# naver/deep-image-retrieval

Measured on AMD Instinct MI355X. Metric: images/sec descriptor extraction (resnet101-GeM, 1024x1024), higher is better.
Workload: dtype fp16p

## Files before the change

### deep-image-retrieval_amd/csrc/c_api.hip

```cpp
#include <initializer_list>
#include <new>

#include "engine.h"
#include "pointwise.h"

namespace dir {
const char* last_error();
}
using namespace dir;

static constexpr int kSimSplitMinRows = 32768;

#define DIR_TRY try {
#define DIR_CATCH                                                   \
    }                                                               \
    catch (const std::bad_alloc&) {                                 \
        return fail(DIR_ERR_NOMEM, "out of host memory");           \
    }                                                               \
    catch (const std::exception& ex) {                              \
        return fail(DIR_ERR_INVALID, std::string("exception: ") + ex.what()); \
    }                                                               \
    catch (...) {                                                   \
        return fail(DIR_ERR_INVALID, "unknown exception");          \
    }
// ... 418 lines not shown
    if (a.ksplit > 1 && conv_splitk_bytes(a, a.ksplit) > scratch_bytes)
        return fail(DIR_ERR_WORKSPACE, "conv: split-K scratch too small");
    if (ksplit_used) *ksplit_used = a.ksplit > 1 ? a.ksplit : 1;
    return conv_launch(a, dtype, variant, (hipStream_t)stream);
    DIR_CATCH
}

static int launch_c3c1(const char* who, const ConvArgs& a, int dtype, void* stream, std::initializer_list<const void*> tensors) {
    for (const void* q : tensors)
        if ((uintptr_t)q & 15) return fail(DIR_ERR_INVALID, std::string(who) + ": tensors must be 16-byte aligned");
    hipError_t e = conv_c3c1_launch(a, dtype, (hipStream_t)stream);
    if (e != hipSuccess) return fail(DIR_ERR_HIP, std::string(who) + " launch: " + hipGetErrorString(e));
    return DIR_OK;
}

int dir_conv_c3c1(const void* t2, const void* w3, const float* bias3, const void* res, void* y, const void* w1,
                  const float* bias1, void* t1, int B, int H, int W, int P, int P2, int relu3, int relu1, int dtype,
                  void* stream) {
    DIR_TRY
    ConvArgs a;
    DIR_CHECK(fill_conv_args(a, t2, w3, bias3, res, y, B, H, W, P, 4 * P, 1, 1, 1, 0, H, W, relu3));
    if (!w1 || !bias1 || !t1 || !res) return fail(DIR_ERR_INVALID, "conv_c3c1: null pointer");
    if (dtype != DIR_BF16 && dtype != DIR_FP16) return fail(DIR_ERR_INVALID, "conv_c3c1: bad dtype");
    conv_args_next_conv1(a, (const uint16_t*)w1, nullptr, bias1, (uint16_t*)t1, P2, relu1 ? 1 : 0);
    if (!conv_c3c1_admissible(a))
        return fail(DIR_ERR_INVALID, "conv_c3c1: planes must be 64, 128 (P2 = P, or 128 after 64) or 256 (P2 = 256, B*H*W % 64 == 0)");
    return launch_c3c1("conv_c3c1", a, dtype, stream, {t2, w3, res, y, w1, t1, bias3, bias1});
    DIR_CATCH
}

int dir_conv_c3c1_ds(const void* t2, const void* x, const void* wcat, const float* bias, void* y, const void* w1,
                     const float* bias1, void* t1, int B, int H, int W, int relu3, int relu1, int dtype,
                     void* stream) {
    DIR_TRY
    ConvArgs a;
    DIR_CHECK(fill_conv_args(a, t2, wcat, bias, nullptr, y, B, H, W, 64, 256, 1, 1, 1, 0, H, W, relu3));
    if (!x || !w1 || !bias1 || !t1) return fail(DIR_ERR_INVALID, "conv_c3c1_ds: null pointer");
    if (dtype != DIR_BF16 && dtype != DIR_FP16) return fail(DIR_ERR_INVALID, "conv_c3c1_ds: bad dtype");
    a.x2 = (const uint16_t*)x;
    a.Cin2 = 64;
    conv_args_next_conv1(a, (const uint16_t*)w1, nullptr, bias1, (uint16_t*)t1, 64, relu1 ? 1 : 0);
    if (!conv_c3c1_admissible(a)) return fail(DIR_ERR_INVALID, "conv_c3c1_ds: shape not admissible");
    return launch_c3c1("conv_c3c1_ds", a, dtype, stream, {t2, x, wcat, y, w1, t1, bias, bias1});
    DIR_CATCH
}

int dir_conv_c3c1_wpair(const void* t2, const void* w3, const void* w3_lo, const float* bias3, const void* res, void* y,
                        const void* w1, const void* w1_lo, const float* bias1, void* t1, int B, int H, int W, int P2,
                        int relu3, int relu1, void* stream) {
    DIR_TRY
    ConvArgs a;
    DIR_CHECK(fill_conv_args(a, t2, w3, bias3, res, y, B, H, W, 64, 256, 1, 1, 1, 0, H, W, relu3));
    if (!w3_lo || !w1 || !bias1 || !t1 || !res) return fail(DIR_ERR_INVALID, "conv_c3c1_wpair: null pointer");
    a.w_lo = (const uint16_t*)w3_lo;
    conv_args_next_conv1(a, (const uint16_t*)w1, (const uint16_t*)w1_lo, bias1, (uint16_t*)t1, P2, relu1 ? 1 : 0);
    if (!conv_c3c1_admissible(a))
        return fail(DIR_ERR_INVALID, "conv_c3c1_wpair: planes 64; P2 = 64 (w1_lo required) or 128 (w1_lo optional)");
    return launch_c3c1("conv_c3c1_wpair", a, DIR_FP16, stream, {t2, w3, w3_lo, res, y, w1, w1_lo, t1, bias3, bias1});
    DIR_CATCH
}

int dir_conv_c3c1_ds_wpair(const void* t2, const void* x, const void* x_lo, const void* wcat, const void* wcat_lo,
                           const float* bias, void* y, const void* w1, const void* w1_lo, const float* bias1, void* t1,
                           int B, int H, int W, int relu3, int relu1, void* stream) {
    DIR_TRY
    ConvArgs a;
    DIR_CHECK(fill_conv_args(a, t2, wcat, bias, nullptr, y, B, H, W, 64, 256, 1, 1, 1, 0, H, W, relu3));
    if (!x || !x_lo || !wcat_lo || !w1 || !w1_lo || !bias1 || !t1) return fail(DIR_ERR_INVALID, "conv_c3c1_ds_wpair: null pointer");
    a.x2 = (const uint16_t*)x;
    a.x2_lo = (const uint16_t*)x_lo;
    a.Cin2 = 64;
    a.w_lo = (const uint16_t*)wcat_lo;
    conv_args_next_conv1(a, (const uint16_t*)w1, (const uint16_t*)w1_lo, bias1, (uint16_t*)t1, 64, relu1 ? 1 : 0);
// ... 473 lines not shown
```

### deep-image-retrieval_amd/csrc/conv_c3c1.hip

```cpp
#include "dir_common.h"
#include "conv_device.h"
#include "conv_igemm.h"

namespace dir {

template <class DT, int P, bool DS, int P2, bool WP3 = false, bool WP1 = false>
__global__ void __launch_bounds__(512) conv_c3c1_kernel(const ConvArgs a) {
    static_assert(P == 64 || P == 128, "planes");
    static_assert(P2 == P || (P == 64 && P2 == 128), "conv1' width");
    static_assert(!DS || (P == 64 && P2 == 64), "the downsample form is layer1's: 64 + 64 input channels");
    static_assert((!WP3 && !WP1) || P == 64, "paired weights: layer1's seams");
    constexpr int KW = P + (DS ? 64 : 0);
    constexpr int KA = KW + (DS && WP3 ? 64 : 0);
    constexpr int C4 = 4 * P;
    constexpr int BM = 64, NT = 512;
    constexpr int CW = C4 / 8;
    constexpr int TA = CW / 32;
    constexpr int KSA = KA / 16;
    constexpr int KSW = KW / 16;
    constexpr int XBUF = BM * KA * 2;
    constexpr int NX = XBUF / 16 / NT;
    constexpr int EROW = 32 * 4 + 16;
    constexpr int EPI_OFF = 2 * XBUF;
    constexpr int OUT_OFF = EPI_OFF + 8 * 32 * EROW;
// ... 103 lines not shown

    u32x4_t xr[NX];
    load_x(tile, xr);
    int cur = 0;
    u32x4_t rres0[TA * 2], rres1[TA * 2];
    if (!DS) load_res(tile, 0, rres0);
    store_x(xr, smem);
    __syncthreads();
    for (;;) {
        const bool more = tile + per < mt;
        const int next = more ? tile + per : tile;
        load_x(next, xr);
        const int m0 = tile * BM;
        if (!DS) load_res(tile, 1, rres1);
        const char* xb = smem + cur * XBUF;

#pragma unroll
        for (int j = 0; j < 2; ++j) {
            f32x16_t acc[TA];
#pragma unroll
            for (int i = 0; i < TA; ++i)
#pragma unroll
                for (int e = 0; e < 16; ++e) acc[i][e] = 0.f;
#pragma unroll
            for (int ks = 0; ks < KSA; ++ks) {
                const frag_t xf = *(const frag_t*)(xb + (ks >> 2) * (BM * 128) + j * (32 * 128) + lbase +
                                                   (((2 * (ks & 3) + lhi) ^ lswz) << 4));
                const int kw = ks < KSW ? ks : ks - 4;
#pragma unroll
                for (int i = 0; i < TA; ++i) {
// ... 25 lines not shown
#pragma unroll
                for (int pass = 0; pass < 2; ++pass) {
                    const int mrow = pass * 16 + erow;
                    const f32x4_t f0 = *(const f32x4_t*)(ebase + mrow * EROW + ecol * 4);
                    const f32x4_t f1 = *(const f32x4_t*)(ebase + mrow * EROW + ecol * 4 + 16);
                    float v[8] = {f0[0] + b0[0], f0[1] + b0[1], f0[2] + b0[2], f0[3] + b0[3],
                                  f1[0] + b1[0], f1[1] + b1[1], f1[2] + b1[2], f1[3] + b1[3]};
                    if (!DS) {
                        const u32x4_t rv = j == 0 ? rres0[i * 2 + pass] : rres1[i * 2 + pass];
                        add_res8<DT>(v, rv);
                    }
                    if (a.relu) relu8(v);
                    u32x4_t ov;
#pragma unroll
                    for (int e = 0; e < 4; ++e) ov[e] = DT::pack(v[2 * e], v[2 * e + 1]);
                    __builtin_amdgcn_raw_buffer_store_b128(ov, rsrc_y, row_off(m0 + j * 32 + mrow), i * 64, 0);
                    ovf.see(ov);
                    const int n = n_wave + i * 32 + ecol, p = j * 32 + mrow;
                    *(u32x4_t*)(otile + (n >> 6) * (BM * 128) + p * 128 + ((((n & 63) >> 3) ^ ((p >> 1) & 7)) << 4)) = ov;
                }
                wave_lds_sync();
            }
            if (!DS && j == 0) load_res(next, 0, rres0);
        }
        __syncthreads();

        {
            constexpr int NJ = WIDE ? 2 : 1;
            f32x16_t acc1[NJ];
#pragma unroll
            for (int jj = 0; jj < NJ; ++jj)
#pragma unroll
                for (int e = 0; e < 16; ++e) acc1[jj][e] = 0.f;
// ... 58 lines not shown
                    ovf.see(ov);
                }
            }
        }
        if (!more) break;
        store_x(xr, smem + (cur ^ 1) * XBUF);
        tile = next;
        cur ^= 1;
        __syncthreads();
    }
    ovf.flush(a.ovf);
}

bool conv_c3c1_admissible(const ConvArgs& a) {
    const bool ds = a.x2 != nullptr;
#ifdef DIR_EXPERIMENTS
    if (a.Cin == 256) return conv_seam3_admissible(a);
#endif
    return a.R == 1 && a.S == 1 && a.stride == 1 && a.pad == 0 && a.H == a.OH && a.W == a.OW &&
           (a.Cin == 64 || a.Cin == 128) && a.Cout == 4 * a.Cin && (ds ? (a.res == nullptr && a.Cin == 64 && a.Cin2 == 64)
                                                                       : a.res != nullptr) &&
           a.w2 != nullptr && a.bias2 != nullptr && a.y2 != nullptr &&
           (a.Cout2 == a.Cin || (!ds && a.Cin == 64 && a.Cout2 == 128)) && (long)a.M * a.Cout < (1L << 30) &&
           ((!a.w_lo && !a.w2_lo && !a.x2_lo) ||
            (a.Cin == 64 && a.w_lo && (a.w2_lo || a.Cout2 == 128) && (ds ? a.x2_lo != nullptr : a.x2_lo == nullptr)));
}

template <class DT, int P, bool DS, int P2 = P, bool WP3 = false, bool WP1 = false>
static hipError_t launch_c3c1(const ConvArgs& a, hipStream_t stream) {
    constexpr int XBUF = 64 * (P + (DS ? 64 : 0) + (DS && WP3 ? 64 : 0)) * 2;
    constexpr int LDS = 2 * XBUF + 8 * 32 * (32 * 4 + 16) + 64 * 4 * P * 2 + (4 * P + P2) * 4;
    static_assert(LDS <= 160 * 1024, "LDS budget");
    auto kern = conv_c3c1_kernel<DT, P, DS, P2, WP3, WP1>;
    static std::atomic<uint64_t> attr_done{0};
    if (hipError_t e = ensure_dynamic_lds((const void*)kern, LDS, attr_done); e != hipSuccess) return e;
    ConvArgs b = a;
    b.x_bytes = (uint32_t)((size_t)a.M * a.Cin * 2);
    const int mt = (a.M + 63) / 64;
    const int ncu = cu_count();
    hipLaunchKernelGGL(kern, dim3(mt < ncu ? mt : ncu), dim3(512), LDS, stream, b);
    return hipGetLastError();
}

hipError_t conv_c3c1_launch(const ConvArgs& a, int dtype, hipStream_t stream) {
#ifdef DIR_EXPERIMENTS
    if (a.Cin == 256) return conv_seam3_launch(a, dtype, stream);
#endif
    if (a.x2 && !env().no_c3c1lc && conv_c3c1ds_lc_admissible(a)) return conv_c3c1ds_lc_launch(a, dtype, stream);
    if (a.w_lo) {
        if (dtype != DIR_FP16) return hipErrorInvalidValue;
        if (a.x2) return a.w2_lo ? launch_c3c1<FP16, 64, true, 64, true, true>(a, stream) : hipErrorInvalidValue;
        if (a.Cout2 == 128)
// ... 15 lines not shown
```

### deep-image-retrieval_amd/csrc/conv_igemm.h

```cpp
#pragma once
#include "dir_common.h"

namespace dir {

struct ConvArgs {
    const uint16_t* x;
    const uint16_t* w;
    const float* bias;
    const uint16_t* res;
    uint16_t* y;
    int B, H, W, Cin, OH, OW, Cout;
    int R, S, stride, pad, relu;
    int M;
    int Ktot;
    int T;
    int ksplit;
    float* partial;
    const uint16_t* w2;
    const float* bias2;
    uint16_t* y2;
    int Cout2, relu2;
    const uint16_t* x2;
    int Cin2;
    int H2, W2, stride2;
// ... 2 lines not shown
    const uint16_t* x_lo;
    const uint16_t* x2_lo;
    const uint16_t* w_lo;
    const uint16_t* w_pw;
    const uint16_t* w_s2;
    const uint16_t* w2_lo;
    const uint16_t* res_lo;
    uint16_t* y_lo;
    int tiles_m, tiles_n;
    uint32_t x_bytes, w_bytes;
    int rev_m;
    int no_xcd_map;
    int flat;
    uint32_t div_ohw_mul, div_ohw_shr;
    uint32_t div_ow_mul, div_ow_shr;
};

inline void fastdiv_init(uint32_t d, uint32_t& mul, uint32_t& shr) {
    if (d <= 1) {
        mul = 0;
        shr = 0;
        return;
    }
    uint32_t l = 0;
    while ((1ull << l) < d) ++l;
    mul = (uint32_t)(((1ull << (31 + l)) + d - 1) / d);
    shr = l - 1;
}

inline void conv_fill_extents(ConvArgs& b) {
// ... 125 lines not shown
```

### deep-image-retrieval_amd/csrc/dir_common.h

```cpp
#pragma once
#include <hip/hip_runtime.h>
#include <stdint.h>
#include <string.h>
#include <atomic>
#include <string>

#include "../../include/dir_engine.h"

namespace dir {

typedef __attribute__((ext_vector_type(8))) __bf16 bf16x8_t;
typedef __attribute__((ext_vector_type(8))) _Float16 f16x8_t;
typedef __attribute__((ext_vector_type(16))) float f32x16_t;
typedef __attribute__((ext_vector_type(4))) float f32x4_t;
typedef __attribute__((ext_vector_type(4))) uint32_t u32x4_t;
typedef __attribute__((ext_vector_type(2))) uint32_t u32x2_t;
typedef __attribute__((ext_vector_type(4))) int i32x4_t;
typedef __attribute__((ext_vector_type(16))) int i32x16_t;
typedef __attribute__((ext_vector_type(2))) float f32x2_t;
typedef __attribute__((ext_vector_type(2))) __bf16 bf16x2_t;
typedef __attribute__((ext_vector_type(2))) _Float16 f16x2_t;

#define DIR_GLOBAL __attribute__((address_space(1)))
#define DIR_LDS __attribute__((address_space(3)))
// ... 23 lines not shown
    bool patchw_pack = false, no_patchw_pack = false;
    bool small_k2 = false;
    bool no_patchs2 = false;
    bool x3_k2048 = false;
    bool lc1x1 = false;
    bool no_c3c1lc = false;
    bool no_smallmap = false;
    bool no_wregd = false;
    bool no_patchw_lc = false;
    bool no_xcdmap = false;
    bool no_pair_patch = false, pair_acts = false;
    int pair_stages = 1;
    bool sim_v1 = false, sim_exact = false;
    bool experiments = false;
    bool no_inplace = false;
    bool no_stem_u8 = false;
    bool stem_pair_old = false;
    bool stem_u8_prep = false;
    bool stem_u8_wg8 = false;
    int stem_u8_seg = 0;
};
const Env& env();
void reload_env();

__host__ __device__ inline uint16_t f32_to_bf16_bits(float f) {
    uint32_t u;
    memcpy(&u, &f, 4);
    if ((u & 0x7fffffffu) > 0x7f800000u) return (uint16_t)((u >> 16) | 0x40);
    u += 0x7fffu + ((u >> 16) & 1u);
    return (uint16_t)(u >> 16);
// ... 149 lines not shown
```

### deep-image-retrieval_amd/csrc/engine.h

```cpp
#pragma once
#include <map>
#include <string>
#include <vector>

#include "conv_f32.h"
#include "conv_igemm.h"
#include "pointwise.h"

namespace dir {

struct HostTensor {
    std::vector<int64_t> shape;
    std::vector<float> data;
};

struct ConvLayer {
    std::string name;
    std::string wkey;
    std::string bnprefix;
    int Cin = 0, Cout = 0, R = 1, S = 1, stride = 1, pad = 0;
    bool relu = false;
    bool stem = false;
    struct Dev {
        uint16_t* w = nullptr;
// ... 88 lines not shown
                int* fh, int* fw, int* fc, void* ws, size_t ws_bytes, hipStream_t stream);
    int forward_f32(const void* img, int B, int H, int W, int fmt, float* desc_out, void* feat_out, int* fh, int* fw,
                    int* fc, char* base, const dir::Plan& p, hipStream_t stream);
    int run_conv_f32(dir::ConvLayer& L, const float* x, const float* res, float* y, int B, int H, int W, int OH, int OW,
                     hipStream_t stream);
    int run_conv(dir::ConvLayer& L, const uint16_t* x, const uint16_t* res, uint16_t* y, int B,
                 int H, int W, int OH, int OW, hipStream_t stream, bool rev_m = false);
    int run_conv_pair(dir::ConvLayer& L, const uint16_t* x, const uint16_t* x_lo, const uint16_t* res,
                      const uint16_t* res_lo, uint16_t* y, uint16_t* y_lo, int B, int H, int W, int OH, int OW,
                      hipStream_t stream, const uint16_t* x2 = nullptr, const uint16_t* x2_lo = nullptr);
    int forward_pair_head(const void* img, int B, int H, int W, int fmt, char* base, const dir::Plan& p,
                          hipStream_t stream, uint16_t** cur, int* h, int* w, size_t* next_block);
    int forward_pair_stem(const void* img, int B, int H, int W, int fmt, char* base, const dir::Plan& p, hipStream_t stream);
    bool pick_seam(const dir::ConvLayer& c3, const dir::ConvLayer& c1, const uint16_t* t2, const uint16_t* res, uint16_t* y,
                   uint16_t* t1, int B, int H, int W, const uint16_t* block_in, const uint16_t* block_in_lo,
                   dir::ConvArgs* a) const;
    int run_seam(const dir::ConvLayer& c3, const dir::ConvLayer& c1, const dir::ConvArgs& a, hipStream_t stream);
    int pick_conv_dual(const dir::ConvLayer& c3, const dir::ConvLayer& ds, const uint16_t* t2, const uint16_t* xin,
                       uint16_t* y, int B, int Hin, int Win, int OH, int OW, dir::ConvArgs* a) const;
    int run_conv_dual(const dir::ConvLayer& c3, const dir::ConvLayer& ds, const dir::ConvArgs& a, int variant,
                      hipStream_t stream);
    int tune_conv(dir::ConvLayer& L, dir::ConvArgs& a, hipStream_t stream, int* variant);
    int finish_descriptor(float* pooled, float* fcout, int B, float* desc_out, hipStream_t stream);
    dir::Env sw;
    float* splitk_scratch = nullptr;
    bool recording() const { return profiling && !prof_paused; }
    int prof_slot(dir::ProfSlot** slot);
    template <class Label, class Launch>
    int profiled(Label&& label, double flops, double bytes, hipStream_t stream, Launch&& launch) {
        if (!recording()) return launch();
        dir::ProfSlot* s = nullptr;
// ... 18 lines not shown
```

### deep-image-retrieval_amd/csrc/engine.hip

```cpp
#include "engine.h"

#include <math.h>
#include <algorithm>

namespace dir {

static thread_local std::string g_err;
void set_error(const std::string& msg) { g_err = msg; }
int fail(int code, const std::string& msg) {
    g_err = msg;
    return code;
}
const char* last_error() { return g_err.c_str(); }


static Env read_env() {
    Env e;
    auto on = [](const char* k) { return getenv(k) != nullptr; };
    const char* mode = getenv("DIRTORCH_AMD_C3C1");
    e.c3c1_off = mode && mode[0] == '0';
    e.c3c1_force = mode && mode[0] == 'f';
    e.no_ds_seam = on("DIRTORCH_AMD_NO_DS_SEAM");
    e.no_dual = on("DIRTORCH_AMD_NO_DUAL");
    e.rev_conv1 = on("DIRTORCH_AMD_REV_CONV1");
// ... 11 lines not shown
    e.small_k2 = on("DIRTORCH_AMD_SMALL_K2");
    e.patchw_pack = on("DIRTORCH_AMD_PATCHW_PACK");
    e.no_patchw_pack = on("DIRTORCH_AMD_NO_PATCHW_PACK");
    e.no_patchw = on("DIRTORCH_AMD_NO_PATCHW");
    e.no_x3 = on("DIRTORCH_AMD_NO_X3");
    e.no_patchs = on("DIRTORCH_AMD_NO_PATCHS");
    e.no_patchw_lc = on("DIRTORCH_AMD_NO_PATCHW_LC");
    e.no_xcdmap = on("DIRTORCH_AMD_NO_XCDMAP");
    e.no_pair_patch = on("DIRTORCH_AMD_NO_PAIR_PATCH");
    e.pair_acts = on("DIRTORCH_AMD_PAIR_ACTS");
    if (const char* s = getenv("DIRTORCH_AMD_PAIR_STAGES")) e.pair_stages = atoi(s);
    e.sim_v1 = on("DIRTORCH_AMD_SIM_V1");
    e.sim_exact = on("DIRTORCH_AMD_SIM_EXACT");
    e.experiments = on("DIRTORCH_AMD_EXPERIMENTS");
    e.no_inplace = on("DIRTORCH_AMD_NO_INPLACE");
    e.no_stem_u8 = on("DIRTORCH_AMD_NO_STEM_U8");
    e.stem_u8_wg8 = on("DIRTORCH_AMD_STEM_U8_WG8");
    e.stem_u8_prep = on("DIRTORCH_AMD_STEM_U8_PREP");
    e.stem_pair_old = on("DIRTORCH_AMD_STEM_PAIR_OLD");
    if (const char* s = getenv("DIRTORCH_AMD_STEM_U8_SEG")) e.stem_u8_seg = atoi(s);
    return e;
}
static Env g_env[2];
static std::atomic<int> g_env_cur{-1};
static std::atomic_flag g_env_lock = ATOMIC_FLAG_INIT;
static void publish_env() {
    while (g_env_lock.test_and_set(std::memory_order_acquire)) {
    }
    const int cur = g_env_cur.load(std::memory_order_relaxed);
    const int nxt = cur < 0 ? 0 : 1 - cur;
// ... 584 lines not shown
        h = oh;
        w = ow;
    }
    *cur_out = pp[cur];
    *h_out = h;
    *w_out = w;
    *next_block = nb;
    return DIR_OK;
}

static constexpr long kSeamMinTiles = 2048;
static constexpr long kSeam3MinTiles = 768;

bool dir_engine::pick_seam(const ConvLayer& c3, const ConvLayer& c1, const uint16_t* t2, const uint16_t* res, uint16_t* y,
                           uint16_t* t1, int B, int H, int W, const uint16_t* block_in, const uint16_t* block_in_lo,
                           ConvArgs* ap) const {
    ConvArgs& a = *ap;
    if (sw.c3c1_off) return false;
    conv_args_init(a, layer_geom(c3, B, H, W, H, W), t2, c3.dev.w, c3.dev.bias, res, y);
    a.w_lo = c3.dev.w_lo;
    if (block_in) {
        if (!c3.dev.w_ds || c3.Cin != 64) return false;
        a.w = c3.dev.w_ds;
        a.w_lo = c3.dev.w_ds_lo;
        a.bias = c3.dev.bias_ds;
        a.res = nullptr;
        a.x2 = block_in;
        a.x2_lo = block_in_lo;
        a.Cin2 = 64;
        if ((c3.dev.w_lo != nullptr) != (a.w_lo != nullptr)) return false;
    }
    conv_args_next_conv1(a, c1.dev.w, c1.dev.w_lo, c1.dev.bias, t1, c1.Cout, c1.relu ? 1 : 0);
    a.ovf = dev.ovf;
    if (c1.R != 1 || c1.S != 1 || c1.stride != 1 || c1.pad != 0 || c1.Cin != c3.Cout || !conv_c3c1_admissible(a))
        return false;
    if (!sw.c3c1_force && (a.M + 63) / 64 < (a.Cin == 256 ? kSeam3MinTiles : kSeamMinTiles)) return false;
    if (a.Cin == 256 && !sw.experiments) return false;
    return true;
}

int dir_engine::run_seam(const ConvLayer& c3, const ConvLayer& c1, const ConvArgs& a, hipStream_t stream) {
    const bool ds = a.x2 != nullptr;
    const double macs = (double)a.M * ((double)c3.Cout * (c3.Cin + a.Cin2) + (double)c1.Cout * c1.Cin);
    const double bytes = 2.0 * ((double)a.M * (c3.Cin + a.Cin2 * (a.x2_lo ? 2 : 1) + (ds ? 1.0 : 2.0) * c3.Cout + c1.Cout) +
                                (double)c3.Cout * (c3.Cin + a.Cin2) * (a.w_lo ? 2 : 1) + (double)c1.Cout * c1.Cin * (a.w2_lo ? 2 : 1));
    return profiled(
        [&](std::string& name, std::string& kernel) {
            name = c3.name.substr(0, c3.name.rfind('.')) + (ds ? ".ds+c3c1" : ".c3c1");
            kernel = (c3.Cin == 256 ? "conv_seam3<" : "conv_c3c1<") + std::to_string(c3.Cin) + (ds ? ",ds" : "") +
                     (a.w_lo ? ",wp>" : ">");
        },
        2.0 * macs, bytes, stream, [&]() -> int {
            hipError_t e = conv_c3c1_launch(a, kdtype(), stream);
            if (e != hipSuccess) return fail(DIR_ERR_HIP, std::string("conv_c3c1 launch: ") + hipGetErrorString(e));
            return DIR_OK;
        });
}

int dir_engine::pick_conv_dual(const ConvLayer& c3, const ConvLayer& ds, const uint16_t* t2, const uint16_t* xin, uint16_t* y,
// ... 81 lines not shown
                               }));
        }
        h = p.PH;
        w = p.PW;
    }

    uint16_t* const pp[2] = {(uint16_t*)(base + p.bufA), (uint16_t*)(base + p.bufB)};
    uint16_t* x4 = nullptr;
    int h4 = 0, w4 = 0;
    bool t1_ready = false;
    for (size_t bi = first_block; bi < blocks.size(); ++bi) {
        BlockDef& bd = blocks[bi];
        const int oh = conv_out(h, 3, bd.stride, 1), ow = conv_out(w, 3, bd.stride, 1);
        const bool keep = (int)bi == x4_block;
        nxt = keep ? (uint16_t*)(base + p.x4) : (cur == pp[0] ? pp[1] : pp[0]);
        if (!sw.no_inplace && desc.bottleneck && bd.down < 0 && !keep && !tuning && convs[bd.conv3].Cin >= 256) nxt = cur;
        const uint16_t* resid = cur;
        const bool seam_next = desc.bottleneck && bi + 1 < blocks.size() && !tuning;
        ConvArgs seam;
        bool ds_in_seam = false;
        if (bd.down >= 0 && seam_next && !sw.no_ds_seam && convs[bd.down].Cin == 64 && convs[bd.down].stride == 1)
            ds_in_seam = pick_seam(convs[bd.conv3], convs[blocks[bi + 1].conv1], t2, nullptr, nxt, t1, B, oh, ow, cur, cur_lo, &seam);
        ConvArgs dual;
        int dual_variant = -1;
        if (bd.down >= 0 && !ds_in_seam && desc.bottleneck && !tuning && !cur_lo)
            dual_variant = pick_conv_dual(convs[bd.conv3], convs[bd.down], t2, cur, nxt, B, h, w, oh, ow, &dual);
        if (bd.down >= 0 && !ds_in_seam && dual_variant < 0) {
            DIR_CHECK(cur_lo ? run_conv_pair(convs[bd.down], cur, cur_lo, nullptr, nullptr, ds, nullptr, B, h, w, oh, ow, stream)
                             : run_conv(convs[bd.down], cur, nullptr, ds, B, h, w, oh, ow, stream));
            resid = ds;
        }
        if (desc.bottleneck) {
            if (!t1_ready)
                DIR_CHECK(cur_lo ? run_conv_pair(convs[bd.conv1], cur, cur_lo, nullptr, nullptr, t1, nullptr, B, h, w, h, w, stream)
                                 : run_conv(convs[bd.conv1], cur, nullptr, t1, B, h, w, h, w, stream, sw.rev_conv1));
            t1_ready = false;
            DIR_CHECK(run_conv(convs[bd.conv2], t1, nullptr, t2, B, h, w, oh, ow, stream));
            if (dual_variant >= 0) {
                DIR_CHECK(run_conv_dual(convs[bd.conv3], convs[bd.down], dual, dual_variant, stream));
            } else if (seam_next && (ds_in_seam || pick_seam(convs[bd.conv3], convs[blocks[bi + 1].conv1], t2, resid, nxt, t1, B, oh,
                                                             ow, nullptr, nullptr, &seam))) {
                DIR_CHECK(run_seam(convs[bd.conv3], convs[blocks[bi + 1].conv1], seam, stream));
                t1_ready = true;
            } else {
                DIR_CHECK(run_conv(convs[bd.conv3], t2, resid, nxt, B, oh, ow, oh, ow, stream, sw.rev_conv3));
            }
        } else {
            DIR_CHECK(run_conv(convs[bd.conv1], cur, nullptr, t1, B, h, w, oh, ow, stream));
            DIR_CHECK(run_conv(convs[bd.conv2], t1, resid, nxt, B, oh, ow, oh, ow, stream));
        }
        cur = nxt;
        cur_lo = nullptr;
        h = oh;
        w = ow;
        if (keep) {
            x4 = cur;
// ... 148 lines not shown
```

### deep-image-retrieval_amd/dirtorch_amd/_lib.py

```python
import ctypes
import os
from ctypes import (POINTER, Structure, c_char, c_char_p, c_double, c_float, c_int, c_int64,
                    c_size_t, c_void_p)

_HERE = os.path.dirname(os.path.abspath(__file__))
LIB_PATH = os.environ.get('DIRTORCH_AMD_LIB') or os.path.join(_HERE, 'libdir_engine.so')

DIR_BF16, DIR_FP16, DIR_F32, DIR_FP16P = 0, 1, 2, 3
DIR_ERR_RANGE = -7
DTYPES = {'bf16': DIR_BF16, 'fp16': DIR_FP16, 'f32': DIR_F32, 'fp16p': DIR_FP16P}
DIR_IMG_F32_NCHW, DIR_IMG_U8_NHWC = 0, 1
DIR_POOL_GEM, DIR_POOL_MAX, DIR_POOL_AVG = 0, 1, 2
POOLING = {'gem': DIR_POOL_GEM, 'max': DIR_POOL_MAX, 'avg': DIR_POOL_AVG}
DIR_HEAD_RMAC, DIR_HEAD_FPN, DIR_HEAD_FPN0, DIR_HEAD_CLASSIFIER = 0, 1, 2, 3


class DirError(RuntimeError):

    def __init__(self, code, msg):
        super().__init__('dir_engine error %d: %s' % (code, msg))
        self.code = code


class ModelDesc(Structure):
# ... 40 lines not shown
                                    c_int, c_int, c_int, c_void_p]),
    'dir_stem_pool_pair': (c_int, [c_void_p] * 7 + [c_int] * 5 + [c_void_p]),
    'dir_stem_pool_u8': (c_int, [c_void_p] * 9 + [c_int] * 4 + [c_void_p]),
    'dir_engine_overflow': (c_int, [c_void_p, c_void_p, POINTER(c_int)]),
    'dir_conv_heuristic': (c_int, [c_int] * 12 + [c_char_p, c_int, POINTER(c_int)]),
    'dir_conv_variant_admissible': (c_int, [c_int] * 13 + [POINTER(c_int)]),
    'dir_conv_variant_splitk': (c_int, [c_int] * 13 + [POINTER(c_int)]),
    'dir_conv_bn_act_splitk': (c_int, [c_void_p, c_void_p, c_void_p, c_void_p, c_void_p] + [c_int] * 15 +
                               [c_void_p, c_size_t, POINTER(c_int), c_void_p]),
    'dir_conv_c3c1': (c_int, [c_void_p, c_void_p, c_void_p, c_void_p, c_void_p, c_void_p, c_void_p, c_void_p]
                      + [c_int] * 8 + [c_void_p]),
    'dir_conv_c3c1_ds': (c_int, [c_void_p, c_void_p, c_void_p, c_void_p, c_void_p, c_void_p, c_void_p, c_void_p]
                         + [c_int] * 6 + [c_void_p]),
    'dir_conv_c3c1_wpair': (c_int, [c_void_p] * 10 + [c_int] * 6 + [c_void_p]),
    'dir_conv_c3c1_ds_wpair': (c_int, [c_void_p] * 11 + [c_int] * 5 + [c_void_p]),
    'dir_conv_dual': (c_int, [c_void_p, c_void_p, c_void_p, c_void_p, c_void_p] + [c_int] * 11 + [c_void_p]),
    'dir_conv_bn_act_naive': (c_int, [c_void_p, c_void_p, c_void_p, c_void_p, c_void_p]
                              + [c_int] * 13 + [c_void_p]),
    'dir_prep_input': (c_int, [c_void_p, c_int, POINTER(c_float), POINTER(c_float), c_void_p,
                               c_int, c_int, c_int, c_int, c_void_p]),
    'dir_stem_pool': (c_int, [c_void_p, c_void_p, c_void_p, c_void_p, c_int, c_int, c_int, c_int, c_int,
                              c_int, c_void_p]),
    'dir_maxpool_3x3s2': (c_int, [c_void_p, c_void_p, c_int, c_int, c_int, c_int, c_int, c_void_p]),
    'dir_global_pool': (c_int, [c_void_p, c_void_p, c_int, c_int, c_int, c_int, c_int, c_float,
                                c_float, c_float, c_int, c_void_p]),
    'dir_resize_workspace_bytes': (c_int, [c_int, c_int, c_int, c_int, c_int, POINTER(c_size_t)]),
    'dir_resize_bilinear_u8': (c_int, [c_void_p, c_void_p, c_int, c_int, c_int, c_int, c_int, c_void_p,
                                       c_size_t, c_void_p]),
    'dir_upsample_add': (c_int, [c_void_p, c_void_p, c_void_p, c_int, c_int, c_int, c_int, c_int,
                                 c_int, c_int, c_void_p]),
# ... 99 lines not shown
```

### deep-image-retrieval_amd/dirtorch_amd/ops.py

```python
import ctypes
import functools

import torch

from . import _lib
from ._lib import DIR_BF16, DIR_FP16, POOLING, call, ptr, stream_ptr


def _dtype_code(t):
    if t.dtype == torch.bfloat16:
        return DIR_BF16
    if t.dtype == torch.float16:
        return DIR_FP16
    raise TypeError('16-bit activation tensor expected (bfloat16 or float16), got %s' % t.dtype)


def _need_cuda(*ts):
    for t in ts:
        if t is not None and not t.is_cuda:
            raise ValueError('device tensor expected')
        if t is not None and not t.is_contiguous():
            raise ValueError('contiguous tensor expected')


# ... 100 lines not shown
    return y, t1


def conv_c3c1_wpair(t2, w3, bias3, res, w1, bias1, relu3=True, relu1=True):
    (w3h, w3l), (w1h, w1l) = w3, w1
    _need_cuda(t2, w3h, w3l, bias3, res, w1h, bias1)
    B, H, W, P = t2.shape
    P2 = w1h.shape[0]
    y = torch.empty(B, H, W, 4 * P, dtype=t2.dtype, device=t2.device)
    t1 = torch.empty(B, H, W, P2, dtype=t2.dtype, device=t2.device)
    call('dir_conv_c3c1_wpair', ptr(t2), ptr(w3h), ptr(w3l), ptr(bias3), ptr(res), ptr(y), ptr(w1h),
         ptr(w1l) if w1l is not None else None, ptr(bias1), ptr(t1), B, H, W, P2, int(bool(relu3)), int(bool(relu1)), stream_ptr())
    return y, t1


def conv_c3c1_ds_wpair(t2, x, wcat, bias, w1, bias1, relu3=True, relu1=True):
    (xh, xl), (wh, wl), (w1h, w1l) = x, wcat, w1
    _need_cuda(t2, xh, xl, wh, wl, bias, w1h, w1l, bias1)
    B, H, W, P = t2.shape
    y = torch.empty(B, H, W, 256, dtype=t2.dtype, device=t2.device)
    t1 = torch.empty(B, H, W, 64, dtype=t2.dtype, device=t2.device)
    call('dir_conv_c3c1_ds_wpair', ptr(t2), ptr(xh), ptr(xl), ptr(wh), ptr(wl), ptr(bias), ptr(y), ptr(w1h), ptr(w1l),
         ptr(bias1), ptr(t1), B, H, W, int(bool(relu3)), int(bool(relu1)), stream_ptr())
    return y, t1


def conv_dual(t2, x, wcat, bias, stride2=2, relu=True):
    _need_cuda(t2, x, wcat, bias)
    B, OH, OW, Cin = t2.shape
    _, H2, W2, Cin2 = x.shape
# ... 690 lines not shown
```

### include/dir_engine.h

```cpp
#ifndef DIR_ENGINE_H
#define DIR_ENGINE_H

#include <stddef.h>
#include <stdint.h>

#ifdef __cplusplus
extern "C" {
#endif

typedef enum dir_status {
    DIR_OK = 0,
    DIR_ERR_INVALID = -1,
    DIR_ERR_STATE = -2,
    DIR_ERR_MISSING = -3,
    DIR_ERR_WORKSPACE = -4,
    DIR_ERR_HIP = -5,
    DIR_ERR_NOMEM = -6,
    DIR_ERR_RANGE = -7
} dir_status;

typedef enum dir_dtype {
    DIR_BF16 = 0,
    DIR_FP16 = 1,
    DIR_F32 = 2,
// ... 100 lines not shown
                           size_t scratch_bytes, int* ksplit_used, void* stream);
int dir_conv_c3c1(const void* t2, const void* w3, const float* bias3, const void* res, void* y, const void* w1,
                  const float* bias1, void* t1, int B, int H, int W, int P, int P2, int relu3, int relu1, int dtype,
                  void* stream);
int dir_conv_dual(const void* t2, const void* x, const void* wcat, const float* bias, void* y, int B, int OH, int OW,
                  int Cin, int Cout, int Cin2, int H2, int W2, int stride2, int relu, int dtype, void* stream);
int dir_conv_c3c1_ds(const void* t2, const void* x, const void* wcat, const float* bias, void* y, const void* w1,
                     const float* bias1, void* t1, int B, int H, int W, int relu3, int relu1, int dtype,
                     void* stream);
int dir_conv_c3c1_wpair(const void* t2, const void* w3, const void* w3_lo, const float* bias3, const void* res, void* y,
                        const void* w1, const void* w1_lo, const float* bias1, void* t1, int B, int H, int W, int P2,
                        int relu3, int relu1, void* stream);
int dir_conv_c3c1_ds_wpair(const void* t2, const void* x, const void* x_lo, const void* wcat, const void* wcat_lo,
                           const float* bias, void* y, const void* w1, const void* w1_lo, const float* bias1, void* t1,
                           int B, int H, int W, int relu3, int relu1, void* stream);
int dir_conv_bn_act_naive(const void* x, const void* w, const float* bias, const void* res,
                          void* y, int B, int H, int W, int Cin, int Cout, int R, int S,
                          int stride, int pad, int OH, int OW, int relu, int dtype, void* stream);
int dir_prep_input(const void* img, int img_format, const float* mean3, const float* std3,
                   void* out, int B, int H, int W, int dtype, void* stream);
int dir_stem_pool(const void* s2d, const void* w, const float* bias, void* y, int B, int H2, int W2,
                  int OH, int OW, int dtype, void* stream);
int dir_resize_workspace_bytes(int B, int H, int W, int OH, int OW, size_t* bytes);
int dir_resize_bilinear_u8(const void* src, void* dst, int B, int H, int W, int OH, int OW,
                           void* workspace, size_t workspace_bytes, void* stream);
int dir_maxpool_3x3s2(const void* x, void* y, int B, int H, int W, int C, int dtype, void* stream);
int dir_global_pool(const void* x, float* out, int B, int H, int W, int C, int pooling, float p,
                    float eps, float center_bias, int dtype, void* stream);
int dir_upsample_add(const void* x, const void* low, void* y, int B, int H, int W, int h, int w, int C,
                     int dtype, void* stream);
// ... 70 lines not shown
```

Before: 2461.

## Store only strided rows of seam output consumed by next strided downsample

In the fused conv3+conv1 seam kernel, the block output y is now written only at positions the next block's strided 1x1 downsample conv will read, when that is the only remaining consumer of the last block before a stage transition. A per-tile ballot mask built with fast division decides which rows are stored, and the rest get an out-of-bounds store offset so the write is dropped. This cuts global write bandwidth for the last layer1/layer2 block outputs. The in-place threshold is also lowered to Cin>=128, so those blocks reuse their input buffer too. The risk is that any other reader of y would see stale data at the skipped positions.

```diff
diff --git a/deep-image-retrieval_amd/csrc/c_api.hip b/deep-image-retrieval_amd/csrc/c_api.hip
--- a/deep-image-retrieval_amd/csrc/c_api.hip
+++ b/deep-image-retrieval_amd/csrc/c_api.hip
@@ -456,18 +456,34 @@
     return DIR_OK;
 }
 
+static int conv_c3c1_entry(const void* t2, const void* w3, const float* bias3, const void* res, void* y, const void* w1,
+                           const float* bias1, void* t1, int B, int H, int W, int P, int P2, int relu3, int relu1,
+                           int keep_stride, int dtype, void* stream) {
+    ConvArgs a;
+    DIR_CHECK(fill_conv_args(a, t2, w3, bias3, res, y, B, H, W, P, 4 * P, 1, 1, 1, 0, H, W, relu3));
+    if (!w1 || !bias1 || !t1 || !res) return fail(DIR_ERR_INVALID, "conv_c3c1: null pointer");
+    if (dtype != DIR_BF16 && dtype != DIR_FP16) return fail(DIR_ERR_INVALID, "conv_c3c1: bad dtype");
+    if (keep_stride < 0) return fail(DIR_ERR_INVALID, "conv_c3c1: negative keep_stride");
+    conv_args_next_conv1(a, (const uint16_t*)w1, nullptr, bias1, (uint16_t*)t1, P2, relu1 ? 1 : 0);
+    a.y_keep_stride = keep_stride;
+    if (!conv_c3c1_admissible(a))
+        return fail(DIR_ERR_INVALID, "conv_c3c1: planes must be 64, 128 (P2 = P, or 128 after 64) or 256 (P2 = 256, B*H*W % 64 == 0; no keep_stride)");
+    return launch_c3c1("conv_c3c1", a, dtype, stream, {t2, w3, res, y, w1, t1, bias3, bias1});
+}
+
 int dir_conv_c3c1(const void* t2, const void* w3, const float* bias3, const void* res, void* y, const void* w1,
                   const float* bias1, void* t1, int B, int H, int W, int P, int P2, int relu3, int relu1, int dtype,
                   void* stream) {
     DIR_TRY
-    ConvArgs a;
-    DIR_CHECK(fill_conv_args(a, t2, w3, bias3, res, y, B, H, W, P, 4 * P, 1, 1, 1, 0, H, W, relu3));
-    if (!w1 || !bias1 || !t1 || !res) return fail(DIR_ERR_INVALID, "conv_c3c1: null pointer");
-    if (dtype != DIR_BF16 && dtype != DIR_FP16) return fail(DIR_ERR_INVALID, "conv_c3c1: bad dtype");
-    conv_args_next_conv1(a, (const uint16_t*)w1, nullptr, bias1, (uint16_t*)t1, P2, relu1 ? 1 : 0);
-    if (!conv_c3c1_admissible(a))
-        return fail(DIR_ERR_INVALID, "conv_c3c1: planes must be 64, 128 (P2 = P, or 128 after 64) or 256 (P2 = 256, B*H*W % 64 == 0)");
-    return launch_c3c1("conv_c3c1", a, dtype, stream, {t2, w3, res, y, w1, t1, bias3, bias1});
+    return conv_c3c1_entry(t2, w3, bias3, res, y, w1, bias1, t1, B, H, W, P, P2, relu3, relu1, 0, dtype, stream);
+    DIR_CATCH
+}
+
+int dir_conv_c3c1_keep(const void* t2, const void* w3, const float* bias3, const void* res, void* y, const void* w1,
+                       const float* bias1, void* t1, int B, int H, int W, int P, int P2, int relu3, int relu1,
+                       int keep_stride, int dtype, void* stream) {
+    DIR_TRY
+    return conv_c3c1_entry(t2, w3, bias3, res, y, w1, bias1, t1, B, H, W, P, P2, relu3, relu1, keep_stride, dtype, stream);
     DIR_CATCH
 }
 
@@ -487,18 +503,35 @@
     DIR_CATCH
 }
 
+static int conv_c3c1_wpair_entry(const void* t2, const void* w3, const void* w3_lo, const float* bias3, const void* res, void* y,
+                                 const void* w1, const void* w1_lo, const float* bias1, void* t1, int B, int H, int W, int P2,
+                                 int relu3, int relu1, int keep_stride, void* stream) {
+    ConvArgs a;
+    DIR_CHECK(fill_conv_args(a, t2, w3, bias3, res, y, B, H, W, 64, 256, 1, 1, 1, 0, H, W, relu3));
+    if (!w3_lo || !w1 || !bias1 || !t1 || !res) return fail(DIR_ERR_INVALID, "conv_c3c1_wpair: null pointer");
+    if (keep_stride < 0) return fail(DIR_ERR_INVALID, "conv_c3c1_wpair: negative keep_stride");
+    a.w_lo = (const uint16_t*)w3_lo;
+    conv_args_next_conv1(a, (const uint16_t*)w1, (const uint16_t*)w1_lo, bias1, (uint16_t*)t1, P2, relu1 ? 1 : 0);
+    a.y_keep_stride = keep_stride;
+    if (!conv_c3c1_admissible(a))
+        return fail(DIR_ERR_INVALID, "conv_c3c1_wpair: planes 64; P2 = 64 (w1_lo required) or 128 (w1_lo optional)");
+    return launch_c3c1("conv_c3c1_wpair", a, DIR_FP16, stream, {t2, w3, w3_lo, res, y, w1, w1_lo, t1, bias3, bias1});
+}
+
 int dir_conv_c3c1_wpair(const void* t2, const void* w3, const void* w3_lo, const float* bias3, const void* res, void* y,
                         const void* w1, const void* w1_lo, const float* bias1, void* t1, int B, int H, int W, int P2,
                         int relu3, int relu1, void* stream) {
     DIR_TRY
-    ConvArgs a;
-    DIR_CHECK(fill_conv_args(a, t2, w3, bias3, res, y, B, H, W, 64, 256, 1, 1, 1, 0, H, W, relu3));
-    if (!w3_lo || !w1 || !bias1 || !t1 || !res) return fail(DIR_ERR_INVALID, "conv_c3c1_wpair: null pointer");
-    a.w_lo = (const uint16_t*)w3_lo;
-    conv_args_next_conv1(a, (const uint16_t*)w1, (const uint16_t*)w1_lo, bias1, (uint16_t*)t1, P2, relu1 ? 1 : 0);
-    if (!conv_c3c1_admissible(a))
-        return fail(DIR_ERR_INVALID, "conv_c3c1_wpair: planes 64; P2 = 64 (w1_lo required) or 128 (w1_lo optional)");
-    return launch_c3c1("conv_c3c1_wpair", a, DIR_FP16, stream, {t2, w3, w3_lo, res, y, w1, w1_lo, t1, bias3, bias1});
+    return conv_c3c1_wpair_entry(t2, w3, w3_lo, bias3, res, y, w1, w1_lo, bias1, t1, B, H, W, P2, relu3, relu1, 0, stream);
+    DIR_CATCH
+}
+
+int dir_conv_c3c1_wpair_keep(const void* t2, const void* w3, const void* w3_lo, const float* bias3, const void* res, void* y,
+                             const void* w1, const void* w1_lo, const float* bias1, void* t1, int B, int H, int W, int P2,
+                             int relu3, int relu1, int keep_stride, void* stream) {
+    DIR_TRY
+    return conv_c3c1_wpair_entry(t2, w3, w3_lo, bias3, res, y, w1, w1_lo, bias1, t1, B, H, W, P2, relu3, relu1, keep_stride,
+                                 stream);
     DIR_CATCH
 }
 
diff --git a/deep-image-retrieval_amd/csrc/conv_c3c1.hip b/deep-image-retrieval_amd/csrc/conv_c3c1.hip
--- a/deep-image-retrieval_amd/csrc/conv_c3c1.hip
+++ b/deep-image-retrieval_amd/csrc/conv_c3c1.hip
@@ -141,6 +141,17 @@
         const int m0 = tile * BM;
         if (!DS) load_res(tile, 1, rres1);
         const char* xb = smem + cur * XBUF;
+        uint64_t ykeep = ~0ull;
+        if (!DS && a.y_keep_stride > 1) {
+            const uint32_t m = (uint32_t)(m0 + lane);
+            const uint32_t img = fast_div(m, a.div_ohw_mul, a.div_ohw_shr);
+            const uint32_t rem = m - img * (uint32_t)(a.H * a.W);
+            const uint32_t row = fast_div(rem, a.div_ow_mul, a.div_ow_shr);
+            const uint32_t col = rem - row * (uint32_t)a.W;
+            const uint32_t s = (uint32_t)a.y_keep_stride;
+            ykeep = __ballot(fast_div(row, a.div_keep_mul, a.div_keep_shr) * s == row &&
+                             fast_div(col, a.div_keep_mul, a.div_keep_shr) * s == col);
+        }
 
 #pragma unroll
         for (int j = 0; j < 2; ++j) {
@@ -196,9 +207,11 @@
                     u32x4_t ov;
 #pragma unroll
                     for (int e = 0; e < 4; ++e) ov[e] = DT::pack(v[2 * e], v[2 * e + 1]);
-                    __builtin_amdgcn_raw_buffer_store_b128(ov, rsrc_y, row_off(m0 + j * 32 + mrow), i * 64, 0);
+                    const int p = j * 32 + mrow;
+                    const uint32_t keep16 = (uint32_t)(ykeep >> (j * 32 + pass * 16));
+                    __builtin_amdgcn_raw_buffer_store_b128(ov, rsrc_y, DS || ((keep16 >> erow) & 1) ? row_off(m0 + p) : kOOB, i * 64, 0);
                     ovf.see(ov);
-                    const int n = n_wave + i * 32 + ecol, p = j * 32 + mrow;
+                    const int n = n_wave + i * 32 + ecol;
                     *(u32x4_t*)(otile + (n >> 6) * (BM * 128) + p * 128 + ((((n & 63) >> 3) ^ ((p >> 1) & 7)) << 4)) = ov;
                 }
                 wave_lds_sync();
@@ -287,6 +300,7 @@
 
 bool conv_c3c1_admissible(const ConvArgs& a) {
     const bool ds = a.x2 != nullptr;
+    if (a.y_keep_stride < 0 || (a.y_keep_stride > 1 && (ds || a.Cin == 256))) return false;
 #ifdef DIR_EXPERIMENTS
     if (a.Cin == 256) return conv_seam3_admissible(a);
 #endif
@@ -309,6 +323,11 @@
     if (hipError_t e = ensure_dynamic_lds((const void*)kern, LDS, attr_done); e != hipSuccess) return e;
     ConvArgs b = a;
     b.x_bytes = (uint32_t)((size_t)a.M * a.Cin * 2);
+    if (a.y_keep_stride > 1) {
+        fastdiv_init((uint32_t)(a.H * a.W), b.div_ohw_mul, b.div_ohw_shr);
+        fastdiv_init((uint32_t)a.W, b.div_ow_mul, b.div_ow_shr);
+        fastdiv_init((uint32_t)a.y_keep_stride, b.div_keep_mul, b.div_keep_shr);
+    }
     const int mt = (a.M + 63) / 64;
     const int ncu = cu_count();
     hipLaunchKernelGGL(kern, dim3(mt < ncu ? mt : ncu), dim3(512), LDS, stream, b);
diff --git a/deep-image-retrieval_amd/csrc/conv_igemm.h b/deep-image-retrieval_amd/csrc/conv_igemm.h
--- a/deep-image-retrieval_amd/csrc/conv_igemm.h
+++ b/deep-image-retrieval_amd/csrc/conv_igemm.h
@@ -40,6 +40,8 @@
     int flat;
     uint32_t div_ohw_mul, div_ohw_shr;
     uint32_t div_ow_mul, div_ow_shr;
+    int y_keep_stride;
+    uint32_t div_keep_mul, div_keep_shr;
 };
 
 inline void fastdiv_init(uint32_t d, uint32_t& mul, uint32_t& shr) {
diff --git a/deep-image-retrieval_amd/csrc/dir_common.h b/deep-image-retrieval_amd/csrc/dir_common.h
--- a/deep-image-retrieval_amd/csrc/dir_common.h
+++ b/deep-image-retrieval_amd/csrc/dir_common.h
@@ -61,6 +61,7 @@
     bool sim_v1 = false, sim_exact = false;
     bool experiments = false;
     bool no_inplace = false;
+    bool seam_full_store = false;
     bool no_stem_u8 = false;
     bool stem_pair_old = false;
     bool stem_u8_prep = false;
diff --git a/deep-image-retrieval_amd/csrc/engine.h b/deep-image-retrieval_amd/csrc/engine.h
--- a/deep-image-retrieval_amd/csrc/engine.h
+++ b/deep-image-retrieval_amd/csrc/engine.h
@@ -126,7 +126,7 @@
     int forward_pair_stem(const void* img, int B, int H, int W, int fmt, char* base, const dir::Plan& p, hipStream_t stream);
     bool pick_seam(const dir::ConvLayer& c3, const dir::ConvLayer& c1, const uint16_t* t2, const uint16_t* res, uint16_t* y,
                    uint16_t* t1, int B, int H, int W, const uint16_t* block_in, const uint16_t* block_in_lo,
-                   dir::ConvArgs* a) const;
+                   dir::ConvArgs* a, int y_keep_stride = 0) const;
     int run_seam(const dir::ConvLayer& c3, const dir::ConvLayer& c1, const dir::ConvArgs& a, hipStream_t stream);
     int pick_conv_dual(const dir::ConvLayer& c3, const dir::ConvLayer& ds, const uint16_t* t2, const uint16_t* xin,
                        uint16_t* y, int B, int Hin, int Win, int OH, int OW, dir::ConvArgs* a) const;
diff --git a/deep-image-retrieval_amd/csrc/engine.hip b/deep-image-retrieval_amd/csrc/engine.hip
--- a/deep-image-retrieval_amd/csrc/engine.hip
+++ b/deep-image-retrieval_amd/csrc/engine.hip
@@ -49,6 +49,7 @@
     e.sim_exact = on("DIRTORCH_AMD_SIM_EXACT");
     e.experiments = on("DIRTORCH_AMD_EXPERIMENTS");
     e.no_inplace = on("DIRTORCH_AMD_NO_INPLACE");
+    e.seam_full_store = on("DIRTORCH_AMD_SEAM_FULL_STORE");
     e.no_stem_u8 = on("DIRTORCH_AMD_NO_STEM_U8");
     e.stem_u8_wg8 = on("DIRTORCH_AMD_STEM_U8_WG8");
     e.stem_u8_prep = on("DIRTORCH_AMD_STEM_U8_PREP");
@@ -663,11 +664,12 @@
 
 bool dir_engine::pick_seam(const ConvLayer& c3, const ConvLayer& c1, const uint16_t* t2, const uint16_t* res, uint16_t* y,
                            uint16_t* t1, int B, int H, int W, const uint16_t* block_in, const uint16_t* block_in_lo,
-                           ConvArgs* ap) const {
+                           ConvArgs* ap, int y_keep_stride) const {
     ConvArgs& a = *ap;
     if (sw.c3c1_off) return false;
     conv_args_init(a, layer_geom(c3, B, H, W, H, W), t2, c3.dev.w, c3.dev.bias, res, y);
     a.w_lo = c3.dev.w_lo;
+    a.y_keep_stride = y_keep_stride;
     if (block_in) {
         if (!c3.dev.w_ds || c3.Cin != 64) return false;
         a.w = c3.dev.w_ds;
@@ -691,7 +693,10 @@
 int dir_engine::run_seam(const ConvLayer& c3, const ConvLayer& c1, const ConvArgs& a, hipStream_t stream) {
     const bool ds = a.x2 != nullptr;
     const double macs = (double)a.M * ((double)c3.Cout * (c3.Cin + a.Cin2) + (double)c1.Cout * c1.Cin);
-    const double bytes = 2.0 * ((double)a.M * (c3.Cin + a.Cin2 * (a.x2_lo ? 2 : 1) + (ds ? 1.0 : 2.0) * c3.Cout + c1.Cout) +
+    const int ks = a.y_keep_stride > 1 ? a.y_keep_stride : 1;
+    const double m_stored = (double)a.B * ((a.H + ks - 1) / ks) * ((a.W + ks - 1) / ks);
+    const double bytes = 2.0 * ((double)a.M * (c3.Cin + a.Cin2 * (a.x2_lo ? 2 : 1) + (ds ? 0.0 : 1.0) * c3.Cout + c1.Cout) +
+                                m_stored * c3.Cout +
                                 (double)c3.Cout * (c3.Cin + a.Cin2) * (a.w_lo ? 2 : 1) + (double)c1.Cout * c1.Cin * (a.w2_lo ? 2 : 1));
     return profiled(
         [&](std::string& name, std::string& kernel) {
@@ -803,9 +808,14 @@
         const int oh = conv_out(h, 3, bd.stride, 1), ow = conv_out(w, 3, bd.stride, 1);
         const bool keep = (int)bi == x4_block;
         nxt = keep ? (uint16_t*)(base + p.x4) : (cur == pp[0] ? pp[1] : pp[0]);
-        if (!sw.no_inplace && desc.bottleneck && bd.down < 0 && !keep && !tuning && convs[bd.conv3].Cin >= 256) nxt = cur;
+        if (!sw.no_inplace && desc.bottleneck && bd.down < 0 && !keep && !tuning && convs[bd.conv3].Cin >= 128) nxt = cur;
         const uint16_t* resid = cur;
         const bool seam_next = desc.bottleneck && bi + 1 < blocks.size() && !tuning;
+        int keep_stride = 0;
+        if (seam_next && !keep && !sw.seam_full_store && bd.down < 0 && blocks[bi + 1].down >= 0 && convs[bd.conv3].Cin <= 128) {
+            const ConvLayer& nd = convs[blocks[bi + 1].down];
+            if (nd.R == 1 && nd.S == 1 && nd.pad == 0 && nd.stride > 1) keep_stride = nd.stride;
+        }
         ConvArgs seam;
         bool ds_in_seam = false;
         if (bd.down >= 0 && seam_next && !sw.no_ds_seam && convs[bd.down].Cin == 64 && convs[bd.down].stride == 1)
@@ -828,7 +838,7 @@
             if (dual_variant >= 0) {
                 DIR_CHECK(run_conv_dual(convs[bd.conv3], convs[bd.down], dual, dual_variant, stream));
             } else if (seam_next && (ds_in_seam || pick_seam(convs[bd.conv3], convs[blocks[bi + 1].conv1], t2, resid, nxt, t1, B, oh,
-                                                             ow, nullptr, nullptr, &seam))) {
+                                                             ow, nullptr, nullptr, &seam, keep_stride))) {
                 DIR_CHECK(run_seam(convs[bd.conv3], convs[blocks[bi + 1].conv1], seam, stream));
                 t1_ready = true;
             } else {
diff --git a/deep-image-retrieval_amd/dirtorch_amd/_lib.py b/deep-image-retrieval_amd/dirtorch_amd/_lib.py
--- a/deep-image-retrieval_amd/dirtorch_amd/_lib.py
+++ b/deep-image-retrieval_amd/dirtorch_amd/_lib.py
@@ -78,6 +78,8 @@
                          + [c_int] * 6 + [c_void_p]),
     'dir_conv_c3c1_wpair': (c_int, [c_void_p] * 10 + [c_int] * 6 + [c_void_p]),
     'dir_conv_c3c1_ds_wpair': (c_int, [c_void_p] * 11 + [c_int] * 5 + [c_void_p]),
+    'dir_conv_c3c1_keep': (c_int, [c_void_p] * 8 + [c_int] * 9 + [c_void_p]),
+    'dir_conv_c3c1_wpair_keep': (c_int, [c_void_p] * 10 + [c_int] * 7 + [c_void_p]),
     'dir_conv_dual': (c_int, [c_void_p, c_void_p, c_void_p, c_void_p, c_void_p] + [c_int] * 11 + [c_void_p]),
     'dir_conv_bn_act_naive': (c_int, [c_void_p, c_void_p, c_void_p, c_void_p, c_void_p]
                               + [c_int] * 13 + [c_void_p]),
diff --git a/deep-image-retrieval_amd/dirtorch_amd/ops.py b/deep-image-retrieval_amd/dirtorch_amd/ops.py
--- a/deep-image-retrieval_amd/dirtorch_amd/ops.py
+++ b/deep-image-retrieval_amd/dirtorch_amd/ops.py
@@ -138,6 +138,39 @@
     return y, t1
 
 
+def _seam_y(y, res):
+    if y is None:
+        return torch.empty_like(res)
+    _need_cuda(y)
+    if y.shape != res.shape or y.dtype != res.dtype:
+        raise ValueError('y must have the shape and dtype of res')
+    return y
+
+
+def conv_c3c1_keep(t2, w3, bias3, res, w1, bias1, keep_stride=0, y=None, relu3=True, relu1=True):
+    _need_cuda(t2, w3, bias3, res, w1, bias1)
+    B, H, W, P = t2.shape
+    P2 = w1.shape[0]
+    y = _seam_y(y, res)
+    t1 = torch.empty(B, H, W, P2, dtype=t2.dtype, device=t2.device)
+    call('dir_conv_c3c1_keep', ptr(t2), ptr(w3), ptr(bias3), ptr(res), ptr(y), ptr(w1), ptr(bias1), ptr(t1), B, H, W, P, P2,
+         int(bool(relu3)), int(bool(relu1)), int(keep_stride), _dtype_code(t2), stream_ptr())
+    return y, t1
+
+
+def conv_c3c1_wpair_keep(t2, w3, bias3, res, w1, bias1, keep_stride=0, y=None, relu3=True, relu1=True):
+    (w3h, w3l), (w1h, w1l) = w3, w1
+    _need_cuda(t2, w3h, w3l, bias3, res, w1h, bias1)
+    B, H, W, P = t2.shape
+    P2 = w1h.shape[0]
+    y = _seam_y(y, res)
+    t1 = torch.empty(B, H, W, P2, dtype=t2.dtype, device=t2.device)
+    call('dir_conv_c3c1_wpair_keep', ptr(t2), ptr(w3h), ptr(w3l), ptr(bias3), ptr(res), ptr(y), ptr(w1h),
+         ptr(w1l) if w1l is not None else None, ptr(bias1), ptr(t1), B, H, W, P2, int(bool(relu3)), int(bool(relu1)),
+         int(keep_stride), stream_ptr())
+    return y, t1
+
+
 def conv_c3c1_ds_wpair(t2, x, wcat, bias, w1, bias1, relu3=True, relu1=True):
     (xh, xl), (wh, wl), (w1h, w1l) = x, wcat, w1
     _need_cuda(t2, xh, xl, wh, wl, bias, w1h, w1l, bias1)
diff --git a/include/dir_engine.h b/include/dir_engine.h
--- a/include/dir_engine.h
+++ b/include/dir_engine.h
@@ -138,6 +138,12 @@
 int dir_conv_c3c1_ds_wpair(const void* t2, const void* x, const void* x_lo, const void* wcat, const void* wcat_lo,
                            const float* bias, void* y, const void* w1, const void* w1_lo, const float* bias1, void* t1,
                            int B, int H, int W, int relu3, int relu1, void* stream);
+int dir_conv_c3c1_keep(const void* t2, const void* w3, const float* bias3, const void* res, void* y, const void* w1,
+                       const float* bias1, void* t1, int B, int H, int W, int P, int P2, int relu3, int relu1,
+                       int keep_stride, int dtype, void* stream);
+int dir_conv_c3c1_wpair_keep(const void* t2, const void* w3, const void* w3_lo, const float* bias3, const void* res, void* y,
+                             const void* w1, const void* w1_lo, const float* bias1, void* t1, int B, int H, int W, int P2,
+                             int relu3, int relu1, int keep_stride, void* stream);
 int dir_conv_bn_act_naive(const void* x, const void* w, const float* bias, const void* res,
                           void* y, int B, int H, int W, int Cin, int Cout, int R, int S,
                           int stride, int pad, int OH, int OW, int relu, int dtype, void* stream);
```

Result: faster. 2488 (median of 6 runs) (+1.1%).
